# wenlinlee/FISCO-BCOS

Measured on AMD Instinct MI355X. Metric: sigs_per_sec, higher is better.
Workload: dtype u32 (256-bit integer); 1 GPU; C2; txs_total=10000, txs_rank0=10000, parallelism=dp1 (tx-index shards)

## Files before the change

fisco-bcos_amd/csrc/ec26_trio.h:

```cpp
#pragma once
#include <type_traits>
#include "ec26.h"

#ifndef TRIO_DUMP
#define TRIO_DUMP(slot, a) ((void)0)
#endif

namespace bcosgpu {

struct TrioPt {
    fe26 S1, Xs, Zs;
    bool inf;
};

struct TrioLane {
    bool r0, r1, r2;
    uint64_t m0, m1, m2, n0, n1, n2;
    F26_HD explicit TrioLane(int lane) {
        const int role = (lane & 15) % 3;
        r0 = role == 0;
        r1 = role == 1;
        r2 = role == 2;
#if defined(__HIP_DEVICE_COMPILE__)
        m0 = __builtin_amdgcn_ballot_w64(r0);
        m1 = __builtin_amdgcn_ballot_w64(r1);
        m2 = __builtin_amdgcn_ballot_w64(r2);
#else
        m0 = m1 = m2 = 0;
#endif
        n0 = ~m0;
        n1 = ~m1;
        n2 = ~m2;
    }
};

#if !defined(__HIP_DEVICE_COMPILE__)
uint32_t trio_emu_dpp(uint32_t x, int ctrl);
bool trio_emu_any(bool b);
#endif

namespace trio {
template <int CTRL>
F26_HD uint32_t dpp(uint32_t x) {
#if defined(__HIP_DEVICE_COMPILE__)
    return static_cast<uint32_t>(__builtin_amdgcn_mov_dpp(static_cast<int>(x), CTRL, 0xf, 0xf, true));
#else
    return trio_emu_dpp(x, CTRL);
#endif
}
F26_HD bool any(bool b) {
#if defined(__HIP_DEVICE_COMPILE__)
    return __any(b);
#else
    return trio_emu_any(b);
#endif
}
constexpr int kL1 = 0x111, kL2 = 0x112, kR1 = 0x101, kR2 = 0x102;

#ifdef FE26_CHECK
template <int CTRL>
F26_HD int mdpp(int m) {
    const int r = static_cast<int>(dpp<CTRL>(static_cast<uint32_t>(m)));
    return r ? r : 1;
}
#endif

template <int CTRL, class E>
F26_HD void fdpp(E& r, const E& a) {
#pragma unroll
    for (int i = 0; i < 10; ++i) r.v[i] = dpp<CTRL>(a.v[i]);
    F26_SETM(r, mdpp<CTRL>(a.m));
}
template <class E>
F26_HD void dpp_fence(E& r) {
#if defined(__HIP_DEVICE_COMPILE__)
    asm volatile("s_nop 1"
                 : "+v"(r.v[0]), "+v"(r.v[1]), "+v"(r.v[2]), "+v"(r.v[3]), "+v"(r.v[4]), "+v"(r.v[5]),
                   "+v"(r.v[6]), "+v"(r.v[7]), "+v"(r.v[8]), "+v"(r.v[9]));
#else
    (void)r;
#endif
}
F26_HD void mul(fe26& r, const fe26& a, const fe26& b) {
    fe26_mul(r, a, b);
    dpp_fence(r);
}
F26_HD void sqr(fe26& r, const fe26& a) {
    fe26_sqr(r, a);
    dpp_fence(r);
}
template <class E>
F26_HD void sel(E& r, bool c, const E& a, const E& b) {
#pragma unroll
    for (int i = 0; i < 10; ++i) r.v[i] = c ? a.v[i] : b.v[i];
    F26_SETM(r, c ? a.m : b.m);
}
template <int C1, int C2, class E>
F26_HD void sel_dpp2(E& r, bool c, const E& a, bool d, const E& b) {
#ifdef FE26_CHECK
    const int m1 = mdpp<C1>(b.m), m2 = mdpp<C2>(b.m);
#endif
#pragma unroll
    for (int i = 0; i < 10; ++i) {
        const uint32_t x = dpp<C1>(b.v[i]), y = dpp<C2>(b.v[i]);
        r.v[i] = c ? a.v[i] : (d ? x : y);
    }
    F26_SETM(r, c ? a.m : d ? m1 : m2);
}
#define TRIO_CSEL_INS(D, S0, S1, CTL) "v_cndmask_b32_dpp %" #D ", %" #S0 ", %" #S1 ", vcc " CTL \
    " row_mask:0xf bank_mask:0xf bound_ctrl:1\n\t"
#define TRIO_CSEL5(CTL, r, a, b, o, cm)                                                                \
    asm volatile("s_mov_b64 vcc, %15\n\ts_nop 1\n\t" TRIO_CSEL_INS(0, 10, 5, CTL) TRIO_CSEL_INS(1, 11, 6, CTL) \
                 TRIO_CSEL_INS(2, 12, 7, CTL) TRIO_CSEL_INS(3, 13, 8, CTL) TRIO_CSEL_INS(4, 14, 9, CTL)      \
                 : "=&v"((r).v[o]), "=&v"((r).v[o + 1]), "=&v"((r).v[o + 2]), "=&v"((r).v[o + 3]),       \
                   "=&v"((r).v[o + 4])                                                                  \
                 : "v"((a).v[o]), "v"((a).v[o + 1]), "v"((a).v[o + 2]), "v"((a).v[o + 3]), "v"((a).v[o + 4]), \
                   "v"((b).v[o]), "v"((b).v[o + 1]), "v"((b).v[o + 2]), "v"((b).v[o + 3]), "v"((b).v[o + 4]), \
                   "s"(cm)                                                                              \
                 : "vcc")
template <int CTRL, class E>
F26_HD void csel(E& r, bool c, uint64_t cm, const E& a, const E& b) {
#if defined(__HIP_DEVICE_COMPILE__)
    (void)c;
    E t;
    if constexpr (CTRL == kL1) {
        TRIO_CSEL5("row_shr:1", t, a, b, 0, cm);
        TRIO_CSEL5("row_shr:1", t, a, b, 5, cm);
    } else if constexpr (CTRL == kL2) {
        TRIO_CSEL5("row_shr:2", t, a, b, 0, cm);
        TRIO_CSEL5("row_shr:2", t, a, b, 5, cm);
    } else if constexpr (CTRL == kR1) {
        TRIO_CSEL5("row_shl:1", t, a, b, 0, cm);
        TRIO_CSEL5("row_shl:1", t, a, b, 5, cm);
    } else {
        static_assert(CTRL == kR2, "csel: row shift by 1 or 2");
        TRIO_CSEL5("row_shl:2", t, a, b, 0, cm);
        TRIO_CSEL5("row_shl:2", t, a, b, 5, cm);
    }
    r = t;
#else
    (void)cm;
#ifdef FE26_CHECK
    const int mb = mdpp<CTRL>(b.m);
#endif
    E t;
#pragma unroll
    for (int i = 0; i < 10; ++i) {
        const uint32_t x = dpp<CTRL>(b.v[i]);
        t.v[i] = c ? a.v[i] : x;
    }
    F26_SETM(t, c ? a.m : mb);
    r = t;
#endif
}
F26_HD uint32_t bdpp_from(uint32_t f, const TrioLane& T, int src) {
    const uint32_t l1 = dpp<kL1>(f), l2 = dpp<kL2>(f), r1 = dpp<kR1>(f), r2 = dpp<kR2>(f);
    if (src == 0) return T.r0 ? f : T.r1 ? l1 : l2;
    if (src == 1) return T.r1 ? f : T.r0 ? r1 : l1;
    return T.r2 ? f : T.r1 ? r1 : r2;
}
}

F26_HD void trio_from_aff(TrioPt& P, const Aff26& Q, const TrioLane& T) {
    trio::sel(P.S1, T.r0, Q.x, Q.y);
    fe26_copy(P.Xs, Q.x);
    fe26_one(P.Zs);
    P.inf = false;
}
F26_HD void trio_set_inf(TrioPt& P) {
    fe26_zero(P.S1);
    fe26_zero(P.Xs);
    fe26_zero(P.Zs);
    P.inf = true;
}
F26_HD void trio_cmov(TrioPt& P, const TrioPt& Q, bool c) {
    fe26_cmov(P.S1, Q.S1, c);
    fe26_cmov(P.Xs, Q.Xs, c);
    fe26_cmov(P.Zs, Q.Zs, c);
    P.inf = c ? Q.inf : P.inf;
}
F26_HD void trio_to_jac(Jac26& J, const TrioPt& P, const TrioLane& T) {
    using namespace trio;
    sel_dpp2<kL1, kL2>(J.X, T.r0, P.S1, T.r1, P.S1);
    sel_dpp2<kR1, kL1>(J.Y, T.r1, P.S1, T.r0, P.S1);
    sel_dpp2<kR1, kR2>(J.Z, T.r2, P.Zs, T.r1, P.Zs);
    J.inf = P.inf;
}

F26_HD void trio_dbl(TrioPt& P, const TrioLane& T) {
    using namespace trio;
    fe26 o1, T2, S2, o2, F, XB, D, X3, W, P3, Q3, o3, C8, Y3, t;
    sqr(o1, P.S1);
#pragma unroll
    for (int i = 0; i < 10; ++i) {
        const uint32_t x3 = (o1.v[i] << 1) + o1.v[i];
        T2.v[i] = T.r0 ? x3 : o1.v[i];
    }
    F26_SETM(T2, T.r0 ? 3 : 1);
    sel(S2, T.r2, P.Xs, T2);
    mul(o2, S2, T2);
    fdpp<kL1>(F, o2);
    fdpp<kR1>(XB, o2);
    fe26_mul_int<4>(D, XB);
    fe26_mul_int<2>(t, D);
    fe26_sub<9>(X3, F, t);
    fe26_sub<11>(W, D, X3);
    csel<kL1>(P3, T.r2, T.m2, P.S1, T2);
    sel(Q3, T.r2, P.Zs, W);
    mul(o3, P3, Q3);
    fe26_mul_int<8>(C8, o2);
    fe26_sub<9>(Y3, o3, C8);
    fe26_mul_int<2>(P.Zs, o3);
    csel<kL1>(t, T.r1, T.m1, Y3, Y3);
    csel<kR1>(P.S1, !T.r0, T.n0, t, X3);
    fdpp<kL1>(P.Xs, X3);
}

template <bool EXC = true>
F26_HD void trio_madd(TrioPt& R, const TrioPt& P, const Aff26& Q, const TrioLane& T) {
    using namespace trio;
    fe26 Zb, P1, o1, P2, Q2, o2, Xl, h, P3, o3, HHx, I, P4, o4, R2, V, X3, W, P5, Q5, o5, Y3, t;
    sel_dpp2<kR1, kR2>(Zb, T.r2, P.Zs, T.r1, P.Zs);
    sel(P1, T.r1, Q.y, Zb);
    mul(o1, P1, Zb);
    TRIO_DUMP(0, o1);
    sel(P2, T.r1, o1, Q.x);
    fdpp<kR1>(Q2, o1);
    sel(Q2, T.r1, Q2, o1);
    mul(o2, P2, Q2);
    TRIO_DUMP(1, o2);
    sel(Xl, T.r2, P.Xs, P.S1);
    fe26_sub<11>(h, o2, Xl);
    sel(P3, T.r2, Zb, h);
    mul(o3, P3, h);
    TRIO_DUMP(2, h);
    TRIO_DUMP(3, o3);
    fdpp<kL2>(HHx, o3);
    sel(HHx, T.r2, HHx, o3);
    fe26_mul_int<4>(I, HHx);
    sel(P4, T.r2, P.Xs, h);
    mul(o4, P4, I);
    TRIO_DUMP(4, o4);
    fdpp<kR1>(R2, o3);
    fe26_mul_int<4>(R2, R2);
    fdpp<kR2>(V, o4);
    fe26_sub<2>(X3, R2, o4);
    fe26_mul_int<2>(t, V);
    fe26_sub<3>(X3, X3, t);
    fe26_sub<10>(W, V, X3);
    fdpp<kR1>(P5, h);
    sel(P5, T.r0, P5, P.S1);
    fdpp<kL1>(Q5, o4);
    sel(Q5, T.r0, W, Q5);
    mul(o5, P5, Q5);
    TRIO_DUMP(5, o5);
    TRIO_DUMP(6, X3);
    fdpp<kR1>(t, o5);
    fe26_sub<2>(Y3, o5, t);
    fe26_mul_int<2>(Y3, Y3);
    TRIO_DUMP(7, Y3);
    TrioPt O;
    sel_dpp2<kL1, kL2>(O.S1, T.r0, X3, T.r1, Y3);
    fdpp<kL2>(O.Xs, X3);
    fe26_mul_int<2>(O.Zs, o3);
    O.inf = false;
    if constexpr (EXC) {
        const uint32_t zf = fe26_is_zero(h) ? 1u : 0u;
        const bool hz = bdpp_from(zf, T, 0) != 0u && !P.inf;
        const bool rz = bdpp_from(zf, T, 1) != 0u;
        if (any(hz && rz)) {
            Jac26 A, D;
            fe26_copy(A.X, P.Xs);
            fe26_copy(A.Y, P.S1);
            fe26_copy(A.Z, P.Zs);
            A.inf = P.inf;
            CurveK1x::dbl(D, A);
            TrioPt Dt;
            sel_dpp2<kR2, kR1>(Dt.S1, T.r2, D.Y, T.r0, D.X);
#pragma unroll
            for (int i = 0; i < 10; ++i) {
                const uint32_t y = dpp<kR1>(D.Y.v[i]);
                Dt.S1.v[i] = T.r1 ? y : Dt.S1.v[i];
            }
            F26_SETM(Dt.S1, 10);
            fe26_copy(Dt.Xs, D.X);
            fe26_copy(Dt.Zs, D.Z);
            Dt.inf = false;
            trio_cmov(O, Dt, hz && rz);
        }
        if (hz && !rz) O.inf = true;
// ... 621 lines not shown
```

fisco-bcos_amd/csrc/ecc_coop.hip:

```cpp
#include "ecc_device.h"
#include "ec26_trio.h"
#include "pair_inv.h"

namespace bcosgpu {

struct SplitLds {
    uint32_t tab[8][16][64];
    uint32_t zc[8][64];
    uint32_t u1[8][64];
    uint32_t k1[4][64];
    uint32_t k2[4][64];
    uint32_t flags[64];
    uint32_t pt[3][25][64];
};

__device__ __forceinline__ void lds_store_jac(uint32_t (*dst)[64], const Jac& P, int lane) {
    lds_store_fe(dst, P.X, lane);
    lds_store_fe(dst + 8, P.Y, lane);
    lds_store_fe(dst + 16, P.Z, lane);
    dst[24][lane] = P.inf ? 1u : 0u;
}
__device__ __forceinline__ void lds_load_jac(Jac& P, const uint32_t (*src)[64], int lane) {
    lds_load_fe(P.X, src, lane);
    lds_load_fe(P.Y, src + 8, lane);
// ... 759 lines not shown
        fe26_mul(V, P.X, I);
        c.puts(3, V);
    }
    __syncthreads();
    if (c.role == 0) c.gets(3, V);
    else c.gets(3, J);
    fe26_sub<2>(X3, R2, J);
    fe26_mul_int<2>(t, V);
    fe26_sub<3>(X3, X3, t);
    if (c.role == 0) {
        fe26_sub<10>(t, V, X3);
        fe26_mul(u, rr, t);
        c.puts(4, u);
    } else {
        fe26_mul(u, P.Y, J);
        c.puts(4, u);
    }
    __syncthreads();
    c.gets(4, t);
    if (c.role == 0) fe26_sub<2>(Y3, u, t);
    else fe26_sub<2>(Y3, t, u);
    fe26_mul_int<2>(Y3, Y3);
    const bool hz = fe26_is_zero(H) && !P.inf;
    const bool rz = fe26_is_zero(rr);
    Jac26 D;
    if (hz && rz) CurveK1x::dbl(D, P);
    const bool pinf = P.inf;
    fe26_copy(R.X, X3);
    fe26_copy(R.Y, Y3);
    fe26_copy(R.Z, Z3);
    R.inf = false;
    if (hz) {
        if (rz) CurveK1x::cmov(R, D, true);
        else R.inf = true;
    }
    if (pinf) {
        fe26_copy(R.X, Q.x);
        fe26_copy(R.Y, Q.y);
        fe26_one(R.Z);
        R.inf = false;
    }
}

__device__ __forceinline__ void coop26_add_digit(Jac26& acc, const Coop26Ctx& c, int d, bool neg, bool phi) {
    const uint32_t m = static_cast<uint32_t>((d < 0 ? -d : d) - 1) & 7u;
    const uint32_t* base = &c.L->tab[0][0][0] + m * (16 * 64) + c.lane;
    const uint32_t* bx = phi ? &c.L->tabphx[0][0][0] + m * (8 * 64) + c.lane : base;
    Aff26 S;
    {
        uint32_t x[8], y[8];
#pragma unroll
        for (int k = 0; k < 8; ++k) {
            x[k] = bx[k * 64];
            y[k] = base[(8 + k) * 64];
        }
        fe26_from_words(S.x, x);
        fe26_from_words(S.y, y);
    }
    fe26 ny;
    fe26_neg<2>(ny, S.y);
    fe26_cmov(S.y, ny, (d < 0) != neg);
    Jac26 R;
    coop26_madd(R, acc, S, c);
    CurveK1x::cmov(acc, R, d != 0);
}


template <int BITS>
__device__ __forceinline__ void comb_range26w(Jac26& acc, const fe& k_plain, const uint32_t* __restrict__ tab, int lo,
                                              int hi) {
    constexpr uint32_t E = 1u << BITS, MASK = E - 1u;
    fe k;
    fe_copy(k, k_plain);
    for (int i = 0; i < lo; ++i) shr_bits<BITS>(k);
    CurveK1x::set_inf(acc);
    uint32_t b = k.v[0] & MASK;
    shr_bits<BITS>(k);
    const uint4* e = reinterpret_cast<const uint4*>(tab + (static_cast<size_t>(lo) * E + b) * 16);
    uint4 q0 = e[0], q1 = e[1], q2 = e[2], q3 = e[3];
#pragma unroll 1
    for (int i = lo; i < hi; ++i) {
        const uint32_t bi = b;
        Aff26 T;
        {
            const uint32_t x[8] = {q0.x, q0.y, q0.z, q0.w, q1.x, q1.y, q1.z, q1.w};
            const uint32_t y[8] = {q2.x, q2.y, q2.z, q2.w, q3.x, q3.y, q3.z, q3.w};
            fe26_from_words(T.x, x);
            fe26_from_words(T.y, y);
        }
        const int in = i + 1 < hi ? i + 1 : i;
        b = k.v[0] & MASK;
        shr_bits<BITS>(k);
        e = reinterpret_cast<const uint4*>(tab + (static_cast<size_t>(in) * E + b) * 16);
        q0 = e[0];
        q1 = e[1];
        q2 = e[2];
        q3 = e[3];
        Jac26 S;
        CurveK1x::madd(S, acc, T);
        CurveK1x::cmov(acc, S, bi != 0u);
    }
}

__device__ __forceinline__ void coop26_store_jac(uint32_t (*dst)[64], const Jac26& P, int lane) {
    fe X, Y, Z;
    fe26_to_fe(X, P.X);
    fe26_to_fe(Y, P.Y);
    fe26_to_fe(Z, P.Z);
    Jac J;
    fe_copy(J.X, X);
    fe_copy(J.Y, Y);
    fe_copy(J.Z, Z);
    J.inf = P.inf;
    coop_store_jac(dst, J, lane);
}
__device__ __forceinline__ void coop26_load_jac(Jac26& P, const uint32_t (*src)[64], int lane) {
    Jac J;
    coop_load_jac(J, src, lane);
    fe26_from_fe(P.X, J.X);
    fe26_from_fe(P.Y, J.Y);
    fe26_from_fe(P.Z, J.Z);
    P.inf = J.inf;
}
__device__ __forceinline__ void lds_load_fe26(fe26& a, const uint32_t (*src)[64], int lane) {
    fe w;
    lds_load_fe(w, src, lane);
    fe26_from_fe(a, w);
}
__device__ __forceinline__ void lds_store_fe26(uint32_t (*dst)[64], const fe26& a, int lane) {
    fe w;
    fe26_to_fe(w, a);
    lds_store_fe(dst, w, lane);
}

constexpr int kTrioWords = 31;
struct Trio26Lds {
    uint32_t tab[8][20][64];
    uint32_t tabphx[8][10][64];
    uint32_t zc[8][64];
    uint32_t k[2][4][64];
    uint32_t flags[64];
    uint32_t pt[5][25][64];
    uint32_t xe[8][64];
    uint32_t xrinv[8][64];
    uint32_t ys[8][64];
    uint32_t rflag[64];
    uint32_t post[3];
};
struct Trio26RecoverLds : Trio26Lds {
    uint32_t sq[10][40];
    uint32_t yok[64];
    uint32_t spost[kTfSlots];
    uint32_t hpost[4];
    uint32_t xg[2][kTrioWords][64];
    uint32_t tsuf[6][10][64];
    uint32_t kw[10][64];
};
__device__ __forceinline__ void lds_flag_wait4(uint32_t* a, uint32_t* b, uint32_t* c, uint32_t* d) {
    for (;;) {
        const uint32_t x = __hip_atomic_load(a, __ATOMIC_RELAXED, __HIP_MEMORY_SCOPE_WORKGROUP);
        const uint32_t y = __hip_atomic_load(b, __ATOMIC_RELAXED, __HIP_MEMORY_SCOPE_WORKGROUP);
        const uint32_t z = __hip_atomic_load(c, __ATOMIC_RELAXED, __HIP_MEMORY_SCOPE_WORKGROUP);
        const uint32_t u = __hip_atomic_load(d, __ATOMIC_RELAXED, __HIP_MEMORY_SCOPE_WORKGROUP);
        if (x != 0u && y != 0u && z != 0u && u != 0u) break;
        __builtin_amdgcn_s_sleep(1);
    }
    __builtin_amdgcn_fence(__ATOMIC_ACQUIRE, "workgroup");
}
struct TrioTableFlags {
    uint32_t* f;
    __device__ __forceinline__ void post(int s) { lds_flag_post(f + s); }
    __device__ __forceinline__ void wait(int s) { lds_flag_wait(f + s); }
    __device__ __forceinline__ void stamp(int k) {
        COOP_T(k);
        (void)k;
    }
};
__device__ __forceinline__ void lds_store_limbs26(uint32_t (*dst)[64], const fe26& a, int lane) {
    fe26 t;
    fe26_copy(t, a);
    fe26_normalize(t);
#pragma unroll
    for (int q = 0; q < 10; ++q) dst[q][lane] = t.v[q];
}

__device__ __forceinline__ void trio_store(uint32_t* buf, const TrioPt& P, int lane) {
#pragma unroll
    for (int q = 0; q < 10; ++q) {
        buf[q * 64 + lane] = P.S1.v[q];
        buf[(10 + q) * 64 + lane] = P.Xs.v[q];
        buf[(20 + q) * 64 + lane] = P.Zs.v[q];
    }
    buf[30 * 64 + lane] = P.inf ? 1u : 0u;
}
__device__ __forceinline__ void trio_load(TrioPt& P, const uint32_t* buf, int lane) {
#pragma unroll
    for (int q = 0; q < 10; ++q) {
        P.S1.v[q] = buf[q * 64 + lane];
        P.Xs.v[q] = buf[(10 + q) * 64 + lane];
        P.Zs.v[q] = buf[(20 + q) * 64 + lane];
    }
    P.inf = buf[30 * 64 + lane] != 0u;
}
__device__ __forceinline__ void trio_from_jac(TrioPt& P, const Jac26& J, const TrioLane& T) {
    trio::sel(P.S1, T.r0, J.X, J.Y);
    fe26_copy(P.Xs, J.X);
    fe26_copy(P.Zs, J.Z);
    P.inf = J.inf;
}

__device__ __forceinline__ void trio_entry(Aff26& S, const Trio26Lds& L, int tl, int d, bool neg, bool phi) {
    const uint32_t m = static_cast<uint32_t>((d < 0 ? -d : d) - 1) & 7u;
    const uint32_t* base = &L.tab[0][0][0] + m * (20 * 64) + tl;
    const uint32_t* bx = phi ? &L.tabphx[0][0][0] + m * (10 * 64) + tl : base;
#pragma unroll
    for (int q = 0; q < 10; ++q) {
        S.x.v[q] = bx[q * 64];
        S.y.v[q] = base[(10 + q) * 64];
    }
    F26_SETM(S.x, 1);
    F26_SETM(S.y, 1);
    fe26 ny;
    fe26_neg<2>(ny, S.y);
    fe26_cmov(S.y, ny, (d < 0) != neg);
}

static constexpr int kTrioLoopPad = 2;
static constexpr int kTrioLoopHeadMod64 = 12;
static_assert(kTrioLoopHeadMod64 == (4 * kTrioLoopPad + 4) % 64, "the pad, then one preheader instruction");

__device__ __forceinline__ void trio_glv_chain(TrioPt& acc, const Trio26Lds& L, int chain, int tl, uint32_t tflags,
                                               const TrioLane& T) {
    fe k;
    fe_zero(k);
#pragma unroll
    for (int q = 0; q < 4; ++q) k.v[q] = L.k[chain][q][tl];
    const bool neg = chain == 0 ? (tflags & 4u) != 0 : (tflags & 8u) != 0;
    const bool phi = chain == 1;
    trio_chain_start(acc, k.v[3], [&](Aff26& S, int d) { trio_entry(S, L, tl, d, neg, phi); }, T);
    shl4_128(k);
    TrioAcc la;
    trio_acc_from(la, acc);
    asm volatile(".p2align 6\n\t.rept %0\n\ts_nop 0\n\t.endr" ::"n"(kTrioLoopPad));
#pragma unroll 1
    for (int w = 30; w >= 0; --w)
        trio_window(la, booth_digit128(k), [&](Aff26& S, int d) { trio_entry(S, L, tl, d, neg, phi); }, T);
    trio_acc_to(acc, la, T);
}

template <bool WITH0, bool WITH2>
__device__ __forceinline__ void trio_sum_partials(TrioPt& A, const Trio26Lds& L, int tl, const TrioLane& T) {
    Jac26 Ga, Gb;
    TrioPt B;
    coop26_load_jac(Ga, L.pt[3], tl);
    coop26_load_jac(Gb, L.pt[4], tl);
    trio_from_jac(A, Ga, T);
    trio_from_jac(B, Gb, T);
    trio_add(A, A, B, T);
    if constexpr (WITH0) {
        coop26_load_jac(Gb, L.pt[0], tl);
        trio_from_jac(B, Gb, T);
        trio_add(A, A, B, T);
    }
    if constexpr (WITH2) {
        coop26_load_jac(Gb, L.pt[2], tl);
        trio_from_jac(B, Gb, T);
        trio_add(A, A, B, T);
    }
}


__device__ __forceinline__ bool recover_w(fe26& X, fe26& w, const fe& r, uint32_t v, bool ok) {
    fe x;
    fe_copy(x, r);
    bool okr = ok;
    if (v & 2u) {
        okr = okr && fe_lt_k(r, kK1PminusN);
        fe_add_k(x, r, ParamN1::M);
    }
    fe26 t, seven;
    fe26_from_fe(X, x);
    fe26_sqr(t, X);
    fe26_mul(w, t, X);
    fe26_set_small(seven, 7u);
    fe26_add(w, w, seven);
    return okr;
}

template <bool LIMBS, class LDS>
__device__ __forceinline__ void coop26_table_to_lds(LDS& L, const Aff26& P, int lane) {
    Aff26 A[8];
    fe26 Zc, beta;
    {
        Jac26 T[8];
        multiples8_26(T, P);
        coz_table26(A, Zc, T);
    }
    fe26_const(beta, kGlvBeta);
    Unroll<0, 8>::run([&](auto J) {
        constexpr int j = decltype(J)::value;
        fe26 bx;
        fe26_mul(bx, A[j].x, beta);
        if constexpr (LIMBS) {
            lds_store_limbs26(L.tab[j], A[j].x, lane);
            lds_store_limbs26(L.tab[j] + 10, A[j].y, lane);
            lds_store_limbs26(L.tabphx[j], bx, lane);
        } else {
            lds_store_fe26(L.tab[j], A[j].x, lane);
            lds_store_fe26(L.tab[j] + 8, A[j].y, lane);
            lds_store_fe26(L.tabphx[j], bx, lane);
        }
    });
    lds_store_fe26(L.zc, Zc, lane);
}

template <bool VERIFY, bool PIPE, class LDS, class IO>
__device__ __forceinline__ void coop26_post_e_inv(LDS& L, const IO& io, uint64_t i, bool active, bool ok, fe& r, fe& s,
                                                  int wave, int lane) {
    if (!ok) {
        fe_zero(r);
        r.v[0] = 1;
        fe_zero(s);
        if (VERIFY) s.v[0] = 1;
    }
    if (wave == 3) {
        fe e;
        fe_zero(e);
        if (active) io.template digest<KECCAK256>(i, e);
        reduce_once(e, ParamN1::M);
        lds_store_fe(L.xe, e, lane);
        lds_flag_post(&L.post[1]);
        COOP_T(7);
    } else if (wave == 0) {
        fe rm, rinv;
        FieldN1::from_plain(rm, VERIFY ? s : r);
        if constexpr (PIPE) FieldInv<FieldN1>::inv_pipe(rinv, rm);
        else FieldInv<FieldN1>::inv(rinv, rm);
        lds_store_fe(L.xrinv, rinv, lane);
        lds_flag_post(&L.post[0]);
        COOP_T(7);
    }
}
template <bool VERIFY, class LDS>
__device__ __forceinline__ void coop26_u1_glv(fe& u1, LDS& L, bool ok, const fe& r, const fe& s, int wave, int lane) {
    lds_flag_wait(&L.post[0]);
    lds_flag_wait(&L.post[1]);
    fe e, rinv;
    lds_load_fe(e, L.xe, lane);
    lds_load_fe(rinv, L.xrinv, lane);
    FieldN1::mul(u1, e, rinv);
    if (!VERIFY) FieldN1::neg(u1, u1);
    if (wave == 1) {
        fe u2, k1, k2;
        FieldN1::mul(u2, VERIFY ? r : s, rinv);
        bool neg1, neg2;
        glv_split(k1, neg1, k2, neg2, u2);
#pragma unroll
        for (int q = 0; q < 4; ++q) {
            L.k[0][q][lane] = k1.v[q];
            L.k[1][q][lane] = k2.v[q];
        }
        L.flags[lane] = (ok ? 1u : 0u) | (neg1 ? 4u : 0u) | (neg2 ? 8u : 0u);
    }
}

struct CombShare {
    int wide[4][2], narrow[4][2];
};
__device__ __forceinline__ void comb_share(int& lo, int& hi, const int (&t)[4][2], int wave) {
    lo = t[0][0];
    hi = t[0][1];
#pragma unroll
    for (int w = 1; w < 4; ++w) {
        if (wave == w) {
            lo = t[w][0];
            hi = t[w][1];
        }
    }
}
__device__ __forceinline__ void comb_share_range(Jac26& G, const fe& u1, const uint32_t* __restrict__ tab, int tab_bits,
                                                 const CombShare& share, int wave) {
    int lo, hi;
    if (tab_bits == kWideBits) {
        comb_share(lo, hi, share.wide, wave);
        comb_range26w<kWideBits>(G, u1, tab, lo, hi);
    } else {
        comb_share(lo, hi, share.narrow, wave);
        comb_range26w<8>(G, u1, tab, lo, hi);
    }
}
constexpr int kPairShare[4][2] = {{0, 12}, {24, 32}, {0, 0}, {12, 24}};
constexpr int kTrioSplitWin[3] = {5, 10, 16};
static_assert(0 < kTrioSplitWin[0] && kTrioSplitWin[0] < kTrioSplitWin[1] && kTrioSplitWin[1] < kTrioSplitWin[2] &&
                  kTrioSplitWin[2] <= 16,
              "comb windows of helpers 0, 1, 3, 2");
constexpr CombShare trio_recover_share() {
    const int a = kTrioSplitWin[0], b = kTrioSplitWin[1], c = kTrioSplitWin[2];
    return {{{0, a}, {a, b}, {c, 16}, {b, c}}, {{0, 2 * a}, {2 * a, 2 * b}, {2 * c, 32}, {2 * b, 2 * c}}};
}
constexpr CombShare kTrioRecoverShare = trio_recover_share();
constexpr CombShare kTrioVerifyShare = {{{0, 6}, {15, 16}, {10, 15}, {6, 10}}, {{0, 11}, {30, 32}, {19, 30}, {11, 19}}};

template <class LDS>
__device__ __forceinline__ void coop26_store_partial(LDS& L, const Jac26& G, int wave, int lane) {
    if (wave == 0) {
        coop26_store_jac(L.pt[2], G, lane);
        lds_flag_post(&L.post[2]);
    } else if (wave == 3) {
        Jac26 G0, S;
        lds_flag_wait(&L.post[2]);
        coop26_load_jac(G0, L.pt[2], lane);
        CurveK1x::add(S, G0, G);
        coop26_store_jac(L.pt[3], S, lane);
    } else {
        coop26_store_jac(L.pt[wave == 1 ? 4 : 0], G, lane);
    }
}

template <class IO>
__device__ __forceinline__ void coop26_body(const IO& io, uint64_t n, const uint32_t* __restrict__ tab) {
    __shared__ Coop26Lds L;
    const int wave = threadIdx.x >> 6, lane = threadIdx.x & 63;
    const uint64_t i = static_cast<uint64_t>(blockIdx.x) * 64 + lane;
    const bool active = i < n;
    COOP_T(0);
    if (threadIdx.x == 0) {
        L.post[0] = 0u;
        L.post[1] = 0u;
        L.post[2] = 0u;
    }
    __syncthreads();
    fe r, s;
    uint32_t v = 0;
    bool ok = false;
    if (active) ok = io.rsv(i, r, s, v);
    else { fe_zero(r); fe_zero(s); }
    if (wave == 1 || wave == 2) {
        fe26 X, rhs;
        bool okr = recover_w(X, rhs, r, v, ok);
        if (wave == 2) {
            fe26 y, ny, t;
            fe26_sqrt_cand(y, rhs);
            fe26_sqr(t, y);
            fe26_sub<3>(t, t, rhs);
            okr = okr && fe26_is_zero(t);
            fe26_normalize(y);
            fe26_neg<2>(ny, y);
            fe26_normalize(ny);
            fe26_cmov(y, ny, (y.v[0] & 1u) != (v & 1u));
            lds_store_fe26(L.ys, y, lane);
            L.rflag[lane] = okr ? 2u : 0u;
            COOP_T(6);
        } else {
            Aff26 R;
            fe26_mul(R.x, rhs, X);
            fe26_sqr(R.y, rhs);
            coop26_table_to_lds<false>(L, R, lane);
            COOP_T(6);
        }
    }
    coop26_post_e_inv<false, false>(L, io, i, active, ok, r, s, wave, lane);
    if (wave != 2) {
        fe u1;
        coop26_u1_glv<false>(u1, L, ok, r, s, wave, lane);
        Jac26 G;
        int lo, hi;
        comb_share(lo, hi, kPairShare, wave);
        comb_range26w<8>(G, u1, tab, lo, hi);
        coop26_store_partial(L, G, wave, lane);
    }
    COOP_T(1);
    __syncthreads();
    const uint32_t flags = L.flags[lane] | L.rflag[lane];
    {
        Coop26Ctx c{&L, wave >> 1, wave & 1, lane, false};
        fe k;
        fe_zero(k);
#pragma unroll
        for (int q = 0; q < 4; ++q) k.v[q] = L.k[c.chain][q][lane];
        const bool neg = c.chain == 0 ? (flags & 4u) != 0 : (flags & 8u) != 0;
        const bool phi = c.chain == 1;
        Jac26 acc;
        CurveK1x::set_inf(acc);
        coop26_add_digit(acc, c, static_cast<int>(k.v[3] >> 31), neg, phi);
#pragma unroll 1
        for (int w = 31; w >= 0; --w) {
            coop26_dbl<0>(acc, c);
#ifdef BCOSGPU_COOP_TIMING
            c.probe = blockIdx.x == 0 && w == 20;
#endif
            coop26_dbl<3>(acc, c);
#ifdef BCOSGPU_COOP_TIMING
            c.probe = false;
            if (blockIdx.x == 0 && w == 20 && (threadIdx.x & 63) == 0) g_dbl_t[threadIdx.x >> 6][5] = clock64();
#endif
            coop26_dbl<0>(acc, c);
            coop26_dbl<3>(acc, c);
#ifdef BCOSGPU_COOP_TIMING
            if (blockIdx.x == 0 && w == 20 && (threadIdx.x & 63) == 0) g_dbl_t[threadIdx.x >> 6][6] = clock64();
#endif
            coop26_add_digit(acc, c, booth_digit128(k), neg, phi);
#ifdef BCOSGPU_COOP_TIMING
            if (blockIdx.x == 0 && w == 20 && (threadIdx.x & 63) == 0) g_dbl_t[threadIdx.x >> 6][7] = clock64();
#endif
        }
        COOP_T(2);
        if (c.role == 0) coop26_store_jac(L.pt[c.chain], acc, lane);
    }
    __syncthreads();
    if (wave == 1) {
        Jac26 G01, G2, U;
        coop26_load_jac(G01, L.pt[3], lane);
        coop26_load_jac(G2, L.pt[4], lane);
        CurveK1x::add(U, G01, G2);
        coop26_store_jac(L.pt[2], U, lane);
    } else if (wave == 0) {
        Jac26 P0, P1, Q;
        coop26_load_jac(P0, L.pt[0], lane);
        coop26_load_jac(P1, L.pt[1], lane);
        fe26 Zc, y;
        lds_load_fe26(Zc, L.zc, lane);
        lds_load_fe26(y, L.ys, lane);
        CurveK1x::add(Q, P0, P1);
        fe26_mul(Zc, Zc, y);
        fe26_mul(Q.Z, Q.Z, Zc);
        coop26_store_jac(L.pt[0], Q, lane);
    }
    __syncthreads();
    if (wave == 0 && active) {
        Jac26 Q, G, R;
        coop26_load_jac(Q, L.pt[0], lane);
        coop26_load_jac(G, L.pt[2], lane);
        CurveK1x::add(R, Q, G);
        const bool ok2 = (flags & 3u) == 3u && !R.inf;
        COOP_T(4);
        fe z, zi, ax, ay;
        fe26_to_fe(z, R.Z);
        FieldInv<FieldK1>::inv(zi, z);
        COOP_T(5);
        fe26 zi26, zi2, zi3, X, Y;
        fe26_from_fe(zi26, zi);
        fe26_sqr(zi2, zi26);
        fe26_mul(X, R.X, zi2);
        fe26_mul(zi3, zi2, zi26);
        fe26_mul(Y, R.Y, zi3);
        fe26_to_fe(ax, X);
        fe26_to_fe(ay, Y);
        uint32_t ad[5] = {0, 0, 0, 0, 0};
        if (ok2 && io.want_addr()) keccak_address(ad, ax, ay);
        io.finish(i, ok2, ad, &ax, &ay);
    }
    COOP_T(3);
}

constexpr int kTrioTxs = 40;
struct TrioSeat {
    int chain, tl;
    bool real;
    __device__ __forceinline__ TrioSeat(int wave, int lane, const TrioLane& T) {
        const int trio_idx = (lane & 15) / 3;
        chain = wave & 1;
        tl = (wave >> 1) * 20 + (lane >> 4) * 5 + (trio_idx < 5 ? trio_idx : 4);
        real = T.r2 && trio_idx < 5;
    }
};

template <class IO>
__device__ __forceinline__ void trio_recover_tail(const IO& io, uint32_t* mbuf, int wave, int lane, const TrioSeat& seat,
                                                  uint64_t ti, bool tactive, bool ok2, const fe& ax, const fe& ay) {
    if (seat.chain == 0 && io.want_addr()) {
        const KeccakPair kp;
        const int j = lane >> 1, t = (wave >> 1) * 20 + (j < 20 ? j : 0);
        uint32_t d[4];
        kp.hash(reinterpret_cast<const uint8_t*>(mbuf + 16 * t), 64u, d);
        if (j < 20) {
#pragma unroll
            for (int q = 0; q < 4; ++q) mbuf[640 + 8 * t + 2 * q + (lane & 1)] = d[q];
        }
    }
    __syncthreads();
    if (seat.chain == 0 && seat.real && tactive) {
        uint32_t ad[5] = {0, 0, 0, 0, 0};
        if (ok2 && io.want_addr()) {
#pragma unroll
            for (int q = 0; q < 5; ++q) ad[q] = mbuf[640 + 8 * seat.tl + 3 + q];
        }
        io.finish(ti, ok2, ad, &ax, &ay);
    }
}

__device__ __forceinline__ void lds_flag_wait_idle(uint32_t* f) {
    while (__hip_atomic_load(f, __ATOMIC_ACQUIRE, __HIP_MEMORY_SCOPE_WORKGROUP) == 0u) __builtin_amdgcn_s_sleep(8);
}

template <class IO>
__device__ __forceinline__ void trio_recover_helper(Trio26RecoverLds& L, const IO& io, uint64_t i, bool active, bool ok,
                                                    const fe& r, uint32_t v, const uint32_t* __restrict__ tab, int tab_bits,
                                                    int h, int lane) {
    constexpr bool kRootAdds = kTrioSplitWin[2] < 16;
    constexpr int kLast = kRootAdds ? 3 : 2;
    if (h == 2) {
        fe26 X, w, y, ny, t;
        const bool okr = recover_w(X, w, r, v, ok);
        fe26_sqrt_cand(y, w);
        fe26_sqr(t, y);
        fe26_sub<3>(t, t, w);
        const bool on = fe26_is_zero(t);
        fe26_normalize(y);
        fe26_neg<2>(ny, y);
        fe26_normalize(ny);
        fe26_cmov(y, ny, (y.v[0] & 1u) != (v & 1u));
        if (lane < kTrioTxs) {
#pragma unroll
            for (int q = 0; q < 10; ++q) L.sq[q][lane] = y.v[q];
        }
        L.rflag[lane] = okr ? 2u : 0u;
        L.yok[lane] = on ? 1u : 0u;
        COOP_T(6);
    } else if (h == 3) {
        fe e;
        fe_zero(e);
        if (active) io.template digest<KECCAK256>(i, e);
        reduce_once(e, ParamN1::M);
        lds_store_fe(L.xe, e, lane);
        lds_flag_post(&L.post[1]);
        COOP_T(7);
    }
    int lo, hi;
    comb_share(lo, hi, kTrioRecoverShare.wide, h);
    if (lo != hi) {
        lds_flag_wait_idle(&L.post[0]);
        lds_flag_wait_idle(&L.post[1]);
        fe e, rinv, u1;
        lds_load_fe(e, L.xe, lane);
        lds_load_fe(rinv, L.xrinv, lane);
        FieldN1::mul(u1, e, rinv);
        FieldN1::neg(u1, u1);
        Jac26 G;
        comb_share_range(G, u1, tab, tab_bits, kTrioRecoverShare, h);
        const int j = h == 0 ? 0 : h == 1 ? 1 : h == 3 ? 2 : 3;
        if (j > 0) {
            Jac26 P, S;
            lds_flag_wait_idle(&L.hpost[j - 1]);
            coop26_load_jac(P, L.pt[j - 1], lane);
            CurveK1x::add(S, P, G);
            coop26_store_jac(L.pt[j == kLast ? 3 : j], S, lane);
        } else {
            coop26_store_jac(L.pt[0], G, lane);
        }
        if (j != kLast) lds_flag_post(&L.hpost[j]);
        COOP_T(10);
    }
}

struct PairOpsTrio {
    const TrioLane& T;
    int lane;
    template <int CTRL>
    __device__ __forceinline__ static void shift(fe& o, const fe& a) {
#pragma unroll
        for (int q = 0; q < 8; ++q) o.v[q] = trio::dpp<CTRL>(a.v[q]);
    }
    __device__ __forceinline__ void right1(fe& o, const fe& a) const { shift<trio::kR1>(o, a); }
    __device__ __forceinline__ void left1(fe& o, const fe& a) const { shift<trio::kL1>(o, a); }
    __device__ __forceinline__ void left2(fe& o, const fe& a) const { shift<trio::kL2>(o, a); }
    __device__ __forceinline__ void sel(fe& o, int roles, const fe& a, const fe& b) const {
        const bool c = ((roles & kPairRole0) && T.r0) || ((roles & kPairRole1) && T.r1) || ((roles & kPairRole2) && T.r2);
#pragma unroll
        for (int q = 0; q < 8; ++q) o.v[q] = c ? a.v[q] : b.v[q];
    }
    __device__ __forceinline__ void mul(fe& o, const fe& a, const fe& b) const {
        FieldN1::mul(o, a, b);
        asm volatile("s_nop 1"
                     : "+v"(o.v[0]), "+v"(o.v[1]), "+v"(o.v[2]), "+v"(o.v[3]), "+v"(o.v[4]), "+v"(o.v[5]), "+v"(o.v[6]),
                       "+v"(o.v[7]));
    }
    __device__ __forceinline__ void inv(fe& o, const fe& x) const {
        fe t, a, b;
        modinv_trio<0, 1>(t, x, kMod30N1, T, lane);
        shift<trio::kR1>(a, t);
        shift<trio::kL1>(b, t);
#pragma unroll
        for (int q = 0; q < 8; ++q) o.v[q] = T.r1 ? t.v[q] : T.r0 ? a.v[q] : b.v[q];
    }
    __device__ __forceinline__ void stamp(int k) const {
        if (k == kPairStampPre) {
            COOP_T(6);
        } else {
            COOP_T(10);
        }
    }
};

template <class IO>
__device__ __forceinline__ void trio26_recover_body(const IO& io, uint64_t n, const uint32_t* __restrict__ tab,
                                                    int tab_bits) {
    __shared__ Trio26RecoverLds L;
    const int wave = __builtin_amdgcn_readfirstlane(static_cast<int>(threadIdx.x >> 6)), lane = threadIdx.x & 63;
    const bool helper = wave >= 4;
    const uint64_t i = static_cast<uint64_t>(blockIdx.x) * kTrioTxs + lane;
    const bool active = lane < kTrioTxs && i < n;
    COOP_T(0);
    if (threadIdx.x == 0) {
        L.post[0] = 0u;
        L.post[1] = 0u;
        L.post[2] = 0u;
#pragma unroll
        for (int q = 0; q < kTfSlots; ++q) L.spost[q] = 0u;
#pragma unroll
        for (int q = 0; q < 4; ++q) L.hpost[q] = 0u;
    }
    __syncthreads();
    const TrioLane T(lane);
    TrioSeat seat(wave, lane, T);
    if (helper) seat.chain = 2;
    const int chain = seat.chain, tl = seat.tl;
    uint32_t tflags = 0;
    TrioPt acc;
    {
        fe r, s;
        uint32_t v = 0;
        bool ok = false;
        fe_zero(r);
        fe_zero(s);
        if (wave != 0 && active && (wave <= 3 || wave == 4 + 2)) ok = io.rsv(i, r, s, v);
        if (helper) {
            trio_recover_helper(L, io, i, active, ok, r, v, tab, tab_bits, wave - 4, lane);
            COOP_T(1);
        } else {
            if (wave == 0) {
                const bool phantom = (lane & 15) == 15, member = !T.r2 && !phantom;
                const int col = phantom ? 60 + (lane >> 4) : tl + (T.r1 ? 20 : T.r2 ? 40 : 0);
                const uint64_t i0 = static_cast<uint64_t>(blockIdx.x) * kTrioTxs + col;
                if (member && i0 < n) ok = io.rsv(i0, r, s, v);
                pair_enter(r, s, ok);
                PairOpsTrio ops{T, lane};
                fe u2, inv, rinv, k1, k2;
                pair_scalars(u2, inv, r, s, ops);
                bool neg1, neg2;
                glv_split(k1, neg1, k2, neg2, u2);
                COOP_T(11);
                if (member) {
#pragma unroll
                    for (int q = 0; q < 4; ++q) {
                        L.k[0][q][col] = k1.v[q];
                        L.k[1][q][col] = k2.v[q];
                    }
                    L.flags[col] = (ok ? 1u : 0u) | (neg1 ? 4u : 0u) | (neg2 ? 8u : 0u);
                }
                lds_flag_post(&L.spost[0]);
                COOP_T(8);
                pair_rinv(rinv, inv, r, ops);
                fe one;
                fe_set(one, ParamN1::ONE);
                fe_cmov(rinv, one, !member);
                lds_store_fe(L.xrinv, rinv, col);
                lds_flag_post(&L.post[0]);
                COOP_T(7);
            } else {
                fe26 X, rhs, beta;
                recover_w(X, rhs, r, v, ok);
                Aff26 R;
                fe26_mul(R.x, rhs, X);
                fe26_sqr(R.y, rhs);
                fe26_const(beta, kGlvBeta);
                TrioTableFlags tf{L.spost};
                if (wave == 1) trio_table_shared<kTableLong>(L, tf, R, rhs, beta, lane);
                else if (wave == 2) trio_table_shared<kTablePrefix>(L, tf, R, rhs, beta, lane);
                else trio_table_shared<kTableShort>(L, tf, R, rhs, beta, lane);
            }
            COOP_T(1);
            lds_flag_wait4(&L.spost[0], &L.spost[kTfDone[kTableLong]], &L.spost[kTfDone[kTablePrefix]],
                           &L.spost[kTfDone[kTableShort]]);
            COOP_T(9);
            tflags = L.flags[tl];
            trio_glv_chain(acc, L, chain, tl, tflags, T);
            COOP_T(2);
        }
    }
    uint32_t* const xbuf = &L.xg[(wave >> 1) & 1][0][0];
    uint32_t* const mbuf = &L.tabphx[0][0][0];
    const uint64_t ti = static_cast<uint64_t>(blockIdx.x) * kTrioTxs + tl;
    const bool tactive = ti < n;
    fe ax, ay;
    bool ok2 = false;
    const auto load_k = [&](fe26& K) {
#pragma unroll
        for (int q = 0; q < 10; ++q) K.v[q] = L.kw[q][tl];
        F26_SETM(K, 1);
    };
    const auto load_g = [&](TrioPt& G) {
        Jac26 J;
        coop26_load_jac(J, L.pt[3], tl);
        trio_from_jac(G, J, T);
    };
    TrioPt SE;
    fe26 zi2, zi3;
    fe26_zero(zi2);
    fe26_zero(zi3);
    if (chain == 1) {
        trio_store(xbuf, acc, lane);
        lds_flag_post(&L.spost[5 + (wave >> 1)]);
    } else if (chain == 0) {
        TrioPt P1;
        lds_flag_wait(&L.spost[5 + (wave >> 1)]);
        trio_load(P1, xbuf, lane);
        trio_add(acc, acc, P1, T);
        trio_store(xbuf, acc, lane);
        fe26 K;
        load_k(K);
        trio_scale_xz(SE, acc, K, T);
    }
    __syncthreads();
    const uint32_t rfl = L.rflag[tl];
    if (chain == 0) {
        TrioPt G;
        load_g(G);
        fe26 Z3;
        trio_add_z(Z3, G, SE, T);
        COOP_T(4);
        fe z, zi;
        fe26_to_fe(z, Z3);
        FieldInv<FieldK1>::inv_trio<2, 2>(zi, z, T, lane);
        COOP_T(5);
        fe26 zi26;
        fe26_from_fe(zi26, zi);
        fe26_sqr(zi2, zi26);
        fe26_mul(zi3, zi2, zi26);
    } else if (chain == 1) {
        TrioPt S, G;
        trio_load(S, xbuf, lane);
        load_g(G);
        fe26 y, zc, K, l;
        load_k(K);
        lds_load_fe26(zc, L.zc, tl);
        trio_scale_xz(SE, S, K, T);
#pragma unroll
        for (int q = 0; q < 10; ++q) y.v[q] = L.sq[q][tl];
        F26_SETM(y, 1);
        COOP_T(4);
        fe26_mul(l, zc, y);
        trio_scale_y(SE, l, T);
        trio_add(S, G, SE, T);
        trio_store(xbuf, S, lane);
        COOP_T(5);
    }
    __syncthreads();
    if (chain == 0) {
        TrioPt O;
        trio_load(O, xbuf, lane);
        ok2 = (tflags & 1u) != 0u && (rfl & 2u) != 0u && L.yok[tl] != 0u && !O.inf;
        fe26 X, Y;
        fe26_mul(X, O.Xs, zi2);
        fe26_mul(Y, O.S1, zi3);
        fe26_to_fe(ax, X);
        fe26_to_fe(ay, Y);
        if (seat.real) {
            uint32_t m[16];
            fe_to_be_words(m, ax);
            fe_to_be_words(m + 8, ay);
#pragma unroll
            for (int q = 0; q < 16; ++q) mbuf[16 * tl + q] = m[q];
        }
    }
    __syncthreads();
    trio_recover_tail(io, mbuf, wave, lane, seat, ti, tactive, ok2, ax, ay);
    COOP_T(3);
}

__device__ __forceinline__ void trio26_verify_body(const KeyIO& io, uint64_t n, const uint32_t* __restrict__ tab,
                                                   int tab_bits) {
    __shared__ Trio26Lds L;
    const int wave = threadIdx.x >> 6, lane = threadIdx.x & 63;
    const uint64_t i = static_cast<uint64_t>(blockIdx.x) * kTrioTxs + lane;
    const bool active = lane < kTrioTxs && i < n;
    COOP_T(0);
    if (threadIdx.x == 0) {
        L.post[0] = 0u;
        L.post[1] = 0u;
        L.post[2] = 0u;
    }
    __syncthreads();
    fe r, s;
    bool ok = false;
    {
        fe kx, ky;
        if (active) {
            io.key_rs(i, r, s, kx, ky);
            ok = fe_lt_k(kx, FieldK1::P) && fe_lt_k(ky, FieldK1::P) && !fe_is_zero_raw(r) && !fe_is_zero_raw(s) &&
                 fe_lt_k(r, ParamN1::M) && fe_lt_k(s, kN1HalfPlus);
        } else {
            fe_zero(r);
            fe_zero(s);
            fe_zero(kx);
            fe_zero(ky);
        }
        if (wave == 0) lds_store_fe(L.ys, r, lane);
        if (wave == 1) {
            Aff26 P;
            fe26_from_fe(P.x, kx);
            fe26_from_fe(P.y, ky);
            fe26 l, rr, t, seven;
            fe26_sqr(l, P.y);
            fe26_sqr(t, P.x);
            fe26_mul(rr, t, P.x);
            fe26_set_small(seven, 7u);
            fe26_add(rr, rr, seven);
            fe26_sub<3>(l, l, rr);
            const bool on = fe26_is_zero(l);
            if (!(ok && on)) {
                fe26_const(P.x, kK1Gx);
                fe26_const(P.y, kK1Gy);
            }
            L.rflag[lane] = on ? 2u : 0u;
            coop26_table_to_lds<true>(L, P, lane);
            COOP_T(6);
        }
    }
    coop26_post_e_inv<true, true>(L, io, i, active, ok, r, s, wave, lane);
    {
        fe u1;
        coop26_u1_glv<true>(u1, L, ok, r, s, wave, lane);
        Jac26 G;
        comb_share_range(G, u1, tab, tab_bits, kTrioVerifyShare, wave);
        coop26_store_partial(L, G, wave, lane);
    }
    COOP_T(1);
    __syncthreads();
    const TrioLane T(lane);
    const TrioSeat seat(wave, lane, T);
    const int chain = seat.chain, tl = seat.tl;
    const uint32_t tflags = L.flags[tl] | L.rflag[tl];
    TrioPt acc;
    trio_glv_chain(acc, L, chain, tl, tflags, T);
    COOP_T(2);
    uint32_t* const xbuf = &L.tab[0][0][0] + (wave >> 1) * kTrioWords * 64;
    uint32_t* const gbuf = &L.tab[0][0][0] + (2 + (wave >> 1)) * kTrioWords * 64;
    const uint64_t ti = static_cast<uint64_t>(blockIdx.x) * kTrioTxs + tl;
    fe26 zcy;
    bool ok2 = false;
    __syncthreads();
    if (chain == 1) trio_store(xbuf, acc, lane);
    else lds_load_fe26(zcy, L.zc, tl);
    __syncthreads();
    if (chain == 1) {
        TrioPt A;
        trio_sum_partials<true, false>(A, L, tl, T);
        trio_store(gbuf, A, lane);
    } else {
        TrioPt P1;
        trio_load(P1, xbuf, lane);
        trio_add(acc, acc, P1, T);
        fe26_mul(acc.Zs, acc.Zs, zcy);
    }
    __syncthreads();
    if (chain == 0) {
        TrioPt G;
        trio_load(G, gbuf, lane);
        trio_add(acc, acc, G, T);
        fe rr, r2, xw, cw;
        lds_load_fe(rr, L.ys, tl);
        fe26 z2, c, rhs;
        fe26_sqr(z2, acc.Zs);
        fe26_from_fe(c, rr);
        fe26_mul(rhs, c, z2);
        fe26_to_fe(xw, acc.Xs);
        fe26_to_fe(cw, rhs);
        bool match = fe_eq_raw(xw, cw);
        const uint32_t carry = fe_add_k(r2, rr, ParamN1::M);
        const bool second = carry == 0u && fe_lt_k(r2, FieldK1::P);
        fe26_from_fe(c, second ? r2 : rr);
        fe26_mul(rhs, c, z2);
        fe26_to_fe(cw, rhs);
        match = match || (second && fe_eq_raw(xw, cw));
        ok2 = (tflags & 3u) == 3u && !acc.inf && match;
    }
    __syncthreads();
    __syncthreads();
    if (chain == 0 && seat.real && ti < n) {
        const uint32_t ad[5] = {0, 0, 0, 0, 0};
        io.finish(ti, ok2, ad, nullptr, nullptr);
    }
    COOP_T(3);
}

template <class IO>
__global__ __launch_bounds__(256, 1) void tx_verify_coop26_kernel(IO io, uint64_t n, const uint32_t* __restrict__ tab) {
    coop26_body(io, n, tab);
}

constexpr int kTrioRecoverThreads = 512;
template <class IO>
__global__ __launch_bounds__(kTrioRecoverThreads, 2) void tx_verify_trio26_kernel(IO io, uint64_t n, const uint32_t* __restrict__ tab,
                                                                  int tab_bits) {
    trio26_recover_body(io, n, tab, tab_bits);
}

__global__ __launch_bounds__(256, 1) void sig_verify_trio26_kernel(KeyIO io, uint64_t n, const uint32_t* __restrict__ tab,
                                                                   int tab_bits) {
    trio26_verify_body(io, n, tab, tab_bits);
}

int launch_sig_verify_small_secp(const KeyIO& io, uint64_t n, hipStream_t st) {
    const uint32_t *k1, *sm2;
// ... 43 lines not shown
```

Baseline: 33.14 million tx/s (hash + recover/verify + sender).

## Replace workgroup barrier in trio recover with per-stage LDS flags and remap helper waves

Removes a __syncthreads between the accumulation and final-add stages of the trio recover kernel. Point-to-point LDS flags now signal when the recovered y and flags, the chain-0 sum, and the last helper partial are ready, so each chain waits only on the data it consumes. Helper waves are remapped so the root/recovery helper runs on wave 7 instead of wave 6. The csel inline asm now binds the mask to vcc through a register variable, dropping the redundant s_mov and second s_nop on the second half. This adds spin-wait polling and ordering risk in exchange for less barrier stall.

```diff
diff --git a/fisco-bcos_amd/csrc/ec26_trio.h b/fisco-bcos_amd/csrc/ec26_trio.h
--- a/fisco-bcos_amd/csrc/ec26_trio.h
+++ b/fisco-bcos_amd/csrc/ec26_trio.h
@@ -109,33 +109,32 @@
 }
 #define TRIO_CSEL_INS(D, S0, S1, CTL) "v_cndmask_b32_dpp %" #D ", %" #S0 ", %" #S1 ", vcc " CTL \
     " row_mask:0xf bank_mask:0xf bound_ctrl:1\n\t"
-#define TRIO_CSEL5(CTL, r, a, b, o, cm)                                                                \
-    asm volatile("s_mov_b64 vcc, %15\n\ts_nop 1\n\t" TRIO_CSEL_INS(0, 10, 5, CTL) TRIO_CSEL_INS(1, 11, 6, CTL) \
+#define TRIO_CSEL5(NOP, CTL, r, a, b, o, cm)                                                            \
+    asm volatile(NOP TRIO_CSEL_INS(0, 10, 5, CTL) TRIO_CSEL_INS(1, 11, 6, CTL)                         \
                  TRIO_CSEL_INS(2, 12, 7, CTL) TRIO_CSEL_INS(3, 13, 8, CTL) TRIO_CSEL_INS(4, 14, 9, CTL)      \
                  : "=&v"((r).v[o]), "=&v"((r).v[o + 1]), "=&v"((r).v[o + 2]), "=&v"((r).v[o + 3]),       \
                    "=&v"((r).v[o + 4])                                                                  \
                  : "v"((a).v[o]), "v"((a).v[o + 1]), "v"((a).v[o + 2]), "v"((a).v[o + 3]), "v"((a).v[o + 4]), \
                    "v"((b).v[o]), "v"((b).v[o + 1]), "v"((b).v[o + 2]), "v"((b).v[o + 3]), "v"((b).v[o + 4]), \
-                   "s"(cm)                                                                              \
-                 : "vcc")
+                   "s"(cm))
+#define TRIO_CSEL10(CTL, r, a, b, cm)                    \
+    register uint64_t vcc_cm asm("vcc") = (cm);          \
+    TRIO_CSEL5("s_nop 1\n\t", CTL, r, a, b, 0, vcc_cm); \
+    TRIO_CSEL5("", CTL, r, a, b, 5, vcc_cm)
 template <int CTRL, class E>
 F26_HD void csel(E& r, bool c, uint64_t cm, const E& a, const E& b) {
 #if defined(__HIP_DEVICE_COMPILE__)
     (void)c;
     E t;
     if constexpr (CTRL == kL1) {
-        TRIO_CSEL5("row_shr:1", t, a, b, 0, cm);
-        TRIO_CSEL5("row_shr:1", t, a, b, 5, cm);
+        TRIO_CSEL10("row_shr:1", t, a, b, cm);
     } else if constexpr (CTRL == kL2) {
-        TRIO_CSEL5("row_shr:2", t, a, b, 0, cm);
-        TRIO_CSEL5("row_shr:2", t, a, b, 5, cm);
+        TRIO_CSEL10("row_shr:2", t, a, b, cm);
     } else if constexpr (CTRL == kR1) {
-        TRIO_CSEL5("row_shl:1", t, a, b, 0, cm);
-        TRIO_CSEL5("row_shl:1", t, a, b, 5, cm);
+        TRIO_CSEL10("row_shl:1", t, a, b, cm);
     } else {
         static_assert(CTRL == kR2, "csel: row shift by 1 or 2");
-        TRIO_CSEL5("row_shl:2", t, a, b, 0, cm);
-        TRIO_CSEL5("row_shl:2", t, a, b, 5, cm);
+        TRIO_CSEL10("row_shl:2", t, a, b, cm);
     }
     r = t;
 #else
diff --git a/fisco-bcos_amd/csrc/ecc_coop.hip b/fisco-bcos_amd/csrc/ecc_coop.hip
--- a/fisco-bcos_amd/csrc/ecc_coop.hip
+++ b/fisco-bcos_amd/csrc/ecc_coop.hip
@@ -935,6 +935,7 @@
     uint32_t yok[64];
     uint32_t spost[kTfSlots];
     uint32_t hpost[4];
+    uint32_t dpost[3];
     uint32_t xg[2][kTrioWords][64];
     uint32_t tsuf[6][10][64];
     uint32_t kw[10][64];
@@ -1182,6 +1183,10 @@
     return {{{0, a}, {a, b}, {c, 16}, {b, c}}, {{0, 2 * a}, {2 * a, 2 * b}, {2 * c, 32}, {2 * b, 2 * c}}};
 }
 constexpr CombShare kTrioRecoverShare = trio_recover_share();
+constexpr int kTrioLastSum = kTrioSplitWin[2] < 16 ? 3 : 2;
+constexpr int trio_helper_of_wave(int wave) { return wave == 6 ? 3 : wave == 7 ? 2 : wave - 4; }
+constexpr int kTrioRootWave = 7;
+static_assert(trio_helper_of_wave(kTrioRootWave) == 2, "the root's helper");
 constexpr CombShare kTrioVerifyShare = {{{0, 6}, {15, 16}, {10, 15}, {6, 10}}, {{0, 11}, {30, 32}, {19, 30}, {11, 19}}};
 
 template <class LDS>
@@ -1380,8 +1385,7 @@
 __device__ __forceinline__ void trio_recover_helper(Trio26RecoverLds& L, const IO& io, uint64_t i, bool active, bool ok,
                                                     const fe& r, uint32_t v, const uint32_t* __restrict__ tab, int tab_bits,
                                                     int h, int lane) {
-    constexpr bool kRootAdds = kTrioSplitWin[2] < 16;
-    constexpr int kLast = kRootAdds ? 3 : 2;
+    constexpr int kLast = kTrioLastSum;
     if (h == 2) {
         fe26 X, w, y, ny, t;
         const bool okr = recover_w(X, w, r, v, ok);
@@ -1399,6 +1403,7 @@
         }
         L.rflag[lane] = okr ? 2u : 0u;
         L.yok[lane] = on ? 1u : 0u;
+        lds_flag_post(&L.dpost[0]);
         COOP_T(6);
     } else if (h == 3) {
         fe e;
@@ -1431,7 +1436,7 @@
         } else {
             coop26_store_jac(L.pt[0], G, lane);
         }
-        if (j != kLast) lds_flag_post(&L.hpost[j]);
+        lds_flag_post(&L.hpost[j]);
         COOP_T(10);
     }
 }
@@ -1492,6 +1497,8 @@
         for (int q = 0; q < kTfSlots; ++q) L.spost[q] = 0u;
 #pragma unroll
         for (int q = 0; q < 4; ++q) L.hpost[q] = 0u;
+#pragma unroll
+        for (int q = 0; q < 3; ++q) L.dpost[q] = 0u;
     }
     __syncthreads();
     const TrioLane T(lane);
@@ -1506,9 +1513,9 @@
         bool ok = false;
         fe_zero(r);
         fe_zero(s);
-        if (wave != 0 && active && (wave <= 3 || wave == 4 + 2)) ok = io.rsv(i, r, s, v);
+        if (wave != 0 && active && (wave <= 3 || wave == kTrioRootWave)) ok = io.rsv(i, r, s, v);
         if (helper) {
-            trio_recover_helper(L, io, i, active, ok, r, v, tab, tab_bits, wave - 4, lane);
+            trio_recover_helper(L, io, i, active, ok, r, v, tab, tab_bits, trio_helper_of_wave(wave), lane);
             COOP_T(1);
         } else {
             if (wave == 0) {
@@ -1590,14 +1597,14 @@
         trio_load(P1, xbuf, lane);
         trio_add(acc, acc, P1, T);
         trio_store(xbuf, acc, lane);
+        lds_flag_post(&L.dpost[1 + (wave >> 1)]);
         fe26 K;
         load_k(K);
         trio_scale_xz(SE, acc, K, T);
     }
-    __syncthreads();
-    const uint32_t rfl = L.rflag[tl];
     if (chain == 0) {
         TrioPt G;
+        lds_flag_wait(&L.hpost[kTrioLastSum]);
         load_g(G);
         fe26 Z3;
         trio_add_z(Z3, G, SE, T);
@@ -1612,12 +1619,16 @@
         fe26_mul(zi3, zi2, zi26);
     } else if (chain == 1) {
         TrioPt S, G;
+        lds_flag_wait(&L.dpost[1 + (wave >> 1)]);
         trio_load(S, xbuf, lane);
+        lds_flag_wait(&L.hpost[kTrioLastSum]);
         load_g(G);
         fe26 y, zc, K, l;
         load_k(K);
         lds_load_fe26(zc, L.zc, tl);
         trio_scale_xz(SE, S, K, T);
+        COOP_T(8);
+        lds_flag_wait(&L.dpost[0]);
 #pragma unroll
         for (int q = 0; q < 10; ++q) y.v[q] = L.sq[q][tl];
         F26_SETM(y, 1);
@@ -1632,7 +1643,7 @@
     if (chain == 0) {
         TrioPt O;
         trio_load(O, xbuf, lane);
-        ok2 = (tflags & 1u) != 0u && (rfl & 2u) != 0u && L.yok[tl] != 0u && !O.inf;
+        ok2 = (tflags & 1u) != 0u && (L.rflag[tl] & 2u) != 0u && L.yok[tl] != 0u && !O.inf;
         fe26 X, Y;
         fe26_mul(X, O.Xs, zi2);
         fe26_mul(Y, O.S1, zi3);
```

Result: faster. 33.90 million tx/s (hash + recover/verify + sender) (median of 6 runs) (+2.3%).
